# KAIST-AILab/SyncVSR

Measured on AMD Instinct MI355X. Metric: lip-clips/sec training (29x88x88), higher is better.
Workload: dtype bf16; 1 GPU; LRW training step (fwd+bwd+allreduce+clip+AdamW), ResNet18 + 6-layer 512-d encoder + vq audio-token CE head, random-init weights, N(0,1) clips 29x88x88, uniform tokens/labels; per_gpu_batch=32, global_batch=32, parallelism=dp1, hip_graph=False, enqueue=native step list

## Files before the change

include/syncvsr_hip.h:

```cpp
#ifndef SYNCVSR_HIP_H
#define SYNCVSR_HIP_H

#include <stdint.h>

#ifndef __HIP_PLATFORM_AMD__
typedef void* hipStream_t;
#else
#include <hip/hip_runtime_api.h>
#endif

#define SVSR_OK 0
#define SVSR_ERR_ARG 1001
#define SVSR_GRAD_ADD_DW 1
#define SVSR_GRAD_ADD_DB 2
#define SVSR_ERR_GROUP_OPEN 1003
#define SVSR_ERR_NO_GROUP 1004
#define SVSR_ERR_MASK_SIZE 1005

typedef struct svsr_wgrad_problem {
    const void* x; const void* dy; float* dw; float* dbias; const int* plan_dev; const int* meta;
    int Nimg; int in_pix; int Ci; int in_pitch; int Co; int out_pix; int out_pitch; int wt_taps;
} svsr_wgrad_problem;

typedef struct svsr_enc_layer {
// ... 23 lines not shown
int svsr_colsum_rows(const float* ws, int nrows, int64_t ld, float* out0, int64_t n0, float* out1, int64_t n1, int accumulate, float scale, hipStream_t stream);
int svsr_colsum_rows_multi(const void* entries, int n, hipStream_t stream);

int svsr_conv_plan(int mode, int Nimg, int H, int W, int Co_out, int k, int stride, int pad, int* words, int cap_words, int* meta);
int svsr_rows_plan(int Nimg, int P, int src0, int dst0, int Co_out, int* words, int cap_words, int* meta);
int svsr_igemm_fwd_kgroups(const int* meta, int Ci, int Co, int bn_epilogue);
int svsr_igemm_fwd(const void* in, const void* wt, void* out, void* out_pre, const float* bias, const void* addend, float* stats, const int* plan_dev, const int* meta, int Nimg, int in_pix, int Ci, int in_pitch, int Co, int out_pix, int out_pitch, int wt_taps, int act, int out_f32, float alpha, const unsigned* drop_seed, unsigned drop_site, float drop_p, hipStream_t stream);

int svsr_wgrad_plan(int Nimg, int H, int W, int Ci, int Co, int k, int stride, int pad, int* words, int cap_words, int* meta, int64_t* part_floats);
int svsr_wgrad_rows_plan(int Nimg, int P, int src0, int dst0, int Ci, int Co, int has_bias, int* words, int cap_words, int* meta, int64_t* part_floats);
int svsr_igemm_wgrad(const void* x, const void* dyp, float* dw, float* dbias, const int* plan_dev, const int* meta, int Nimg, int in_pix, int Ci, int in_pitch, int Co, int out_pix, int out_pitch, int wt_taps, float* part, int64_t part_floats, hipStream_t stream);
int svsr_wgrad_rows_plan_tile(int Nimg, int P, int src0, int dst0, int Ci, int Co, int has_bias, int bc, int* words, int cap_words, int* meta, int64_t* part_floats);
int64_t svsr_igemm_wgrad_group_bytes(int n);
int svsr_igemm_wgrad_group(const svsr_wgrad_problem* problems, int n, void* table_dev, int64_t table_bytes, hipStream_t stream);
int svsr_igemm_wgrad_v2(const void* x, const void* dyp, float* dw, float* dbias, const int* plan_dev, const int* meta, int Nimg, int in_pix, int Ci, int in_pitch, int Co, int out_pix, int out_pitch, int wt_taps, float* part, int64_t part_floats, int mode, hipStream_t stream);
int svsr_igemm_wgrad_group_v2(const svsr_wgrad_problem* problems, const int* modes, int n, void* table_dev, int64_t table_bytes, hipStream_t stream);

int svsr_conv3x3_c64_stat_rows(int Nimg, int H, int W);
int64_t svsr_conv3x3_c64_pixtab(int Nimg, int H, int W, int* out, int64_t cap);
int svsr_conv3x3_c64(const void* in, const void* wt, void* out, const void* addend, float* stats, int Nimg, int H, int W, const int* dy, const int* dx, const int* tw, const int* pixtab, hipStream_t stream);

int svsr_igemm_dgrad_bn(const void* in, const void* wt, void* out, const void* addend, float* stats, const int* plan_dev, const int* meta, int Nimg, int in_pix, int Ci, int in_pitch, int Co, int out_pix, int out_pitch, int wt_taps, const void* y, const void* x, const float* mean, const float* rstd, const float* gamma, const float* beta, int act, hipStream_t stream);
int svsr_igemm_dgrad_relu(const void* in, const void* wt, void* out, float* stats, const int* plan_dev, const int* meta, int Nimg, int in_pix, int Ci, int in_pitch, int Co, int out_pix, int out_pitch, int wt_taps, const void* y, const float* zeros, const float* ones, float gscale, hipStream_t stream);
int svsr_conv3x3_c64_dgrad_bn(const void* in, const void* wt, void* out, const void* addend, float* stats, int Nimg, int H, int W, const int* dy, const int* dx, const int* tw, const void* y, const void* x, const float* mean, const float* rstd, const float* gamma, const float* beta, int act, const int* pixtab, hipStream_t stream);
int svsr_bn_bwd_from_stats(const void* g, const void* x, const float* mean, const float* rstd, const float* gamma, const float* stats, int nrows, float* coef, float* dgamma, float* dbeta, void* dx, int64_t npix, int C, hipStream_t stream);


int svsr_conv3x3_wgrad_plan(int Nimg, int H, int W, int Ci, int Co, int* splits, int64_t* part_floats);
int svsr_conv3x3_wgrad(const void* x, const void* dy, float* dw, int Nimg, int H, int W, int Ci, int Co, float* part, int64_t part_floats, hipStream_t stream);
int svsr_conv3x3_wgrad_v2(const void* x, const void* dy, float* dw, int Nimg, int H, int W, int Ci, int Co, float* part, int64_t part_floats, int mode, hipStream_t stream);
int svsr_conv3x3_wgrad_chain(const void* x, const void* dy, float* dw, int Nimg, int H, int W, int Ci, int Co, float* part, int64_t part_floats, int mode, int defer, const float* pend_part, float* pend_dw, int pend_splits, int pend_Ci, int pend_Co, int pend_mode, hipStream_t stream);
int svsr_conv3x3_wgrad_reduce(const float* part, float* dw, int splits, int Ci, int Co, int mode, hipStream_t stream);

int svsr_stem_conv_fwd_stat_rows(int B, int T, int H, int W);
int64_t svsr_stem_conv_fwd_ws_bytes(int B, int T, int H, int W);
int svsr_stem_conv_fwd(const float* vid, const float* w, void* out, float* stats, int B, int T, int H, int W, void* ws, int64_t ws_bytes, hipStream_t stream);

int svsr_stem_conv_wgrad_plan(int B, int T, int H, int W, int* splits, int64_t* part_floats);
int svsr_stem_conv_wgrad(const float* vid, const void* dy, float* dw, int B, int T, int H, int W, int use_tr, float* part, int64_t part_floats, hipStream_t stream);

int svsr_stem_bwd_wgrad_ok(int B, int T, int H, int W);
int svsr_stem_bwd_wgrad(const float* vid, const void* gpool, const void* amax, const void* x, const float* mean, const float* rstd, const float* coef, float* dw, int B, int T, int H, int W, float* part, int64_t part_floats, hipStream_t stream);

int svsr_bn_finalize(const float* part, int nrows, int C, float count, float eps, float momentum, float* mean, float* rstd, float* running_mean, float* running_var, int64_t* num_batches_tracked, hipStream_t stream);

int svsr_bn_eval_prepare(const float* running_mean, const float* running_var, int C, float eps, float* mean, float* rstd, hipStream_t stream);
// ... 197 lines not shown
```

syncvsr_amd/csrc/igemm_fwd.h:

```cpp
#pragma once
#include "common.h"

struct IgemmFwdArgs {
    const bf16_t* in;
    const bf16_t* wt;
    void* out;
    bf16_t* out_pre;
    const float* bias;
    const bf16_t* addend;
    float* stats;
    const int* plan;
    int Nimg, in_pix, Ci, in_pitch;
    int Co, out_pix, out_pitch, wt_taps;
    int act, out_f32;
    float alpha;
    DropArgs drop;
    const bf16_t* bnb_y;
    const bf16_t* bnb_x;
    const float* bnb_mean;
    const float* bnb_rstd;
    const float* bnb_gamma;
    const float* bnb_beta;
    int bnb_act;
};


#define LDS_SWZ(row, chunk) ((row) * 64 + ((((chunk) ^ (((row) >> 1) & 7))) << 3))

#define P8_MAGIC 0x50380001
#define P8_HDR_WORDS 8
#define P8_DESC_WORDS 64
#define P8_BM 256
#define P8_BN 128
int igemm_p8_launch(const IgemmFwdArgs& a, const int* meta, hipStream_t stream);
```

syncvsr_amd/csrc/igemm_fwd.hip:

```cpp

#include <algorithm>
#include <map>
#include <vector>

#include "common.h"
#include "igemm_fwd.h"

#define PLAN_CLS_WORDS 24
#define PLAN_HDR_WORDS 2

__device__ unsigned g_zero_page[64];


template <int BM, int BN, int TM, int TN>
__device__ __forceinline__ void igemm_epilogue(const IgemmFwdArgs& p, f32x16 (&acc)[TM][TN], unsigned char* smem_raw, const long* sRow,
                                               int wm0, int wn0, int n0, int tid, bool active, int m_tile) {
    constexpr int WN = BN / 2;
    const int lane = tid & 63, wave = tid >> 6;
    float st_s[TN], st_q[TN];
    const bool bnb = p.bnb_x != nullptr;
    if (p.stats != nullptr && !bnb) {
#pragma unroll
        for (int j = 0; j < TN; ++j) {
            float s = 0.f, q = 0.f;
// ... 268 lines not shown
        for (int i = 0; i < TM; ++i)
#pragma unroll
            for (int j = 0; j < TN; ++j)
                acc[i][j] = __builtin_amdgcn_mfma_f32_32x32x16_bf16(fa[i], fb[j], acc[i][j], 0, 0, 0);
    }
}

template <int LPT, int MAXL>
__device__ __forceinline__ void wait_tiles_barrier(int later) {
    if constexpr (MAXL > 0) {
        if (later == MAXL) { SVSR_WAIT_VM_BARRIER(LPT * MAXL); return; }
        wait_tiles_barrier<LPT, MAXL - 1>(later);
    } else {
        asm volatile("s_waitcnt vmcnt(0)\n\ts_barrier" ::: "memory");
    }
}

__device__ __forceinline__ void split_row(int m, int P, float inv_p, int& n, int& j) {
    n = (int)((float)m * inv_p);
    j = m - n * P;
    if (j < 0) { n--; j += P; } else if (j >= P) { n++; j -= P; }
}

template <int BM, int BN, int NS, int KG = 1>
__global__ __launch_bounds__(256 * KG) void k_igemm_fwd_glds(const IgemmFwdArgs p) {
    constexpr int BK = 64;
    static_assert(NS >= 2 && (BM / 32 + BN / 32) * (NS - 2) <= 63, "vmcnt immediate is 6 bits");
    constexpr int WM = BM / 2, WN = BN / 2, TM = WM / 32, TN = WN / 32;
    constexpr int A_ELEMS = BM * BK, B_ELEMS = BN * BK, S_ELEMS = A_ELEMS + B_ELEMS;
    constexpr int AR = BM / 32, BR = BN / 32, LPT = AR + BR;
    extern __shared__ __attribute__((aligned(16))) unsigned char smem_raw[];
    const int grp = KG == 1 ? 0 : __builtin_amdgcn_readfirstlane((int)threadIdx.x >> 8);
    bf16_t* sStage = reinterpret_cast<bf16_t*>(smem_raw) + grp * NS * S_ELEMS;
    long* sRow = reinterpret_cast<long*>(reinterpret_cast<bf16_t*>(smem_raw) + KG * NS * S_ELEMS);
    int* sTap = reinterpret_cast<int*>(sRow + BM);

    const int tid = threadIdx.x & 255, lane = tid & 63, wave = tid >> 6;
    const int wm0 = (wave >> 1) * WM, wn0 = (wave & 1) * WN;
    const int bx = blockIdx.x, by = blockIdx.y;
    const int n0 = by * BN;
    const int slot = tid & 7, r0 = tid >> 3;
    const int csw = slot ^ ((r0 >> 1) & 7);
    const int wrow = __builtin_amdgcn_readfirstlane(wave) * 8;

    const int hdr0 = p.plan[0];
    const int ncls = hdr0 & 0xffff;
    const bool identity = (hdr0 >> 16) != 0;
// ... 32 lines not shown
    }
    for (int r = tid; r < BM; r += 256) {
        const int m = m0 + r;
        long off = -1;
        if (m < Mc) {
            if (identity) {
                off = (long)m * p.out_pix * p.out_pitch;
            } else {
                int n, j;
                split_row(m, P, inv_p, n, j);
                off = ((long)n * p.out_pix + pos[2 * j + 1]) * p.out_pitch;
            }
        }
        sRow[r] = off;
    }
    __syncthreads();

    const int KT_all = ntaps * (p.Ci / BK);
    const int KT_loop = (KT_all + KG - 1) / KG;
    const int k_begin = grp * KT_loop;
    const int KT = KT_all - k_begin < KT_loop ? (KT_all - k_begin > 0 ? KT_all - k_begin : 0) : KT_loop;
    const int spt = p.Ci / BK;
    int t_next = k_begin / spt, c_next = (k_begin - (k_begin / spt) * spt) * BK;
    auto stage = [&](int buf) {
        const int tw = sTap[9 + t_next];
        const int c0 = c_next;
        const long a_off = (long)sTap[t_next] * p.in_pitch + c0;
        bf16_t* dstA = sStage + buf * S_ELEMS + wrow * 64;
#pragma unroll
        for (int i = 0; i < AR; ++i) {
            const bf16_t* src = ((a_ok >> i) & 1u) ? a_ptr[i] + a_off : zero_src;
            __builtin_amdgcn_global_load_lds((const __attribute__((address_space(1))) void*)src,
                                             (__attribute__((address_space(3))) void*)(dstA + i * 32 * 64), 16, 0, 0);
        }
        bf16_t* dstB = sStage + buf * S_ELEMS + A_ELEMS + wrow * 64;
#pragma unroll
        for (int i = 0; i < BR; ++i) {
            const bf16_t* src = b_ptr[i] != nullptr ? b_ptr[i] + (long)tw * p.Ci + c0 : zero_src;
            __builtin_amdgcn_global_load_lds((const __attribute__((address_space(1))) void*)src,
                                             (__attribute__((address_space(3))) void*)(dstB + i * 32 * 64), 16, 0, 0);
        }
        c_next += BK;
        if (c_next >= p.Ci) { c_next = 0; ++t_next; }
    };

    f32x16 acc[TM][TN];
#pragma unroll
    for (int i = 0; i < TM; ++i)
#pragma unroll
        for (int j = 0; j < TN; ++j)
#pragma unroll
            for (int r = 0; r < 16; ++r) acc[i][j][r] = 0.f;

#pragma unroll
    for (int s = 0; s < NS - 1; ++s)
        if (s < KT) stage(s);
    int buf = 0;
    for (int it = 0; it < KT_loop; ++it) {
        int later = KT - 1 - it < NS - 2 ? KT - 1 - it : NS - 2;
        if (later < 0) later = 0;
        wait_tiles_barrier<LPT, NS - 2>(later);
        if (it + NS - 1 < KT) stage(buf >= 1 ? buf - 1 : NS - 1);
        if (KG == 1 || it < KT) {
            const bf16_t* cA = sStage + buf * S_ELEMS;
            igemm_mma_tile<BM, BN, TM, TN>(cA, cA + A_ELEMS, acc, wm0, wn0, lane);
        }
// ... 5 lines not shown
        static_assert((size_t)TM * TN * 16 * 256 * sizeof(float) <= (size_t)NS * S_ELEMS * sizeof(bf16_t), "exchange buffer fits the ring");
        if (grp == 1) {
#pragma unroll
            for (int i = 0; i < TM; ++i)
#pragma unroll
                for (int j = 0; j < TN; ++j)
#pragma unroll
                    for (int r = 0; r < 16; ++r) sX[((i * TN + j) * 16 + r) * 256 + tid] = acc[i][j][r];
        }
        __syncthreads();
        if (grp == 0) {
#pragma unroll
            for (int i = 0; i < TM; ++i)
#pragma unroll
                for (int j = 0; j < TN; ++j)
#pragma unroll
                    for (int r = 0; r < 16; ++r) acc[i][j][r] += sX[((i * TN + j) * 16 + r) * 256 + tid];
        }
        __syncthreads();
    }
    igemm_epilogue<BM, BN, TM, TN>(p, acc, smem_raw, sRow, wm0, wn0, n0, tid, grp == 0, bx);
}

template <int BM, int BN, int NS, int KG = 1>
static int launch_glds(const IgemmFwdArgs& a, int gx, int gy, hipStream_t stream) {
    const size_t lds = (size_t)KG * NS * (BM + BN) * 64 * sizeof(bf16_t) + (size_t)BM * sizeof(long) + 128;
    static size_t attr_set = 0;
    if (attr_set < lds) {
        (void)hipFuncSetAttribute(reinterpret_cast<const void*>(k_igemm_fwd_glds<BM, BN, NS, KG>), hipFuncAttributeMaxDynamicSharedMemorySize, (int)lds);
        attr_set = lds;
    }
    IgemmFwdArgs b = a;
    hipLaunchKernelGGL((k_igemm_fwd_glds<BM, BN, NS, KG>), dim3(gx, gy), dim3(256 * KG), lds, stream, b);
    return svsr_check_launch();
}

struct IgemmFwdPlan { int bm, bn, ns, gy; };

static IgemmFwdPlan igemm_fwd_plan(long M, int Co, int max_taps) {
    const int cus = svsr_stream_cus(nullptr);
    IgemmFwdPlan pl;
    const int forced = svsr_tune_get(SVSR_TUNE_IGEMM_TILE);
    const int thr = svsr_tune_get(SVSR_TUNE_IGEMM_M128);
    int bm;
    if (forced == 64 || forced == 128) bm = forced;
    else if (Co <= 64) bm = M >= 16384 ? 128 : 64;
    else {
        const long blocks128 = ((M + 127) / 128) * ((Co + 127) / 128);
        bm = (M >= thr || blocks128 >= 224) ? 128 : 64;
    }
    const int lin_rows = svsr_tune_get(SVSR_TUNE_IGEMM_LIN_BN64);
    if (bm == 64 && forced == 0 && Co > 64 && max_taps == 1 && lin_rows > 0 && M >= lin_rows) { pl.bm = 128; pl.bn = 64; pl.ns = 3; }
    else if (bm == 128 && Co > 64 && max_taps > 1 && ((M + 127) / 128) * ((Co + 127) / 128) < svsr_tune_get(SVSR_TUNE_IGEMM_BN64_BELOW)) { pl.bm = 128; pl.bn = 64; pl.ns = 2; }
    else if (bm == 128 && Co <= 64) { pl.bm = 128; pl.bn = 64; pl.ns = max_taps <= 4 ? 2 : 3; }
    else if (bm == 128) { pl.bm = 128; pl.bn = 128; pl.ns = 2; }
    else { pl.bm = 64; pl.bn = 64; pl.ns = 0; }
// ... 72 lines not shown
            const PlanClass& c = cls[i];
            int* w = words + PLAN_HDR_WORDS + i * PLAN_CLS_WORDS;
            const int P = (int)(c.pos.size() / 2);
            if ((long)Nimg * P >= (1L << 24)) return -SVSR_ERR_ARG;
            w[0] = c.ntaps; w[1] = P; w[2] = pos_off; w[3] = (int)tiles;
            for (int t = 0; t < 9; ++t) { w[4 + t] = t < c.ntaps ? c.delta[t] : 0; w[13 + t] = t < c.ntaps ? c.tw[t] : 0; }
            w[22] = 0; w[23] = 0;
            std::copy(c.pos.begin(), c.pos.end(), words + pos_word0 + 2 * pos_off);
            pos_off += P;
            tiles += ((long)Nimg * P + pl.bm - 1) / pl.bm;
        }
    } else {
        for (const PlanClass& c : cls) tiles += ((long)Nimg * (long)(c.pos.size() / 2) + pl.bm - 1) / pl.bm;
    }
    if (tiles > 0x7fffffffL) return -SVSR_ERR_ARG;
    if (meta != nullptr) {
        meta[0] = pl.bm; meta[1] = pl.bn; meta[2] = pl.ns; meta[3] = (int)tiles; meta[4] = pl.gy; meta[5] = ncls; meta[6] = max_taps;
        meta[7] = (int)(M & 0x7fffffff);
    }
    return nwords;
}

extern "C" int svsr_conv_plan(int mode, int Nimg, int H, int W, int Co_out, int k, int stride, int pad, int* words, int cap_words, int* meta) {
    if (Nimg < 1 || H < 1 || W < 1 || k < 1 || k > 3 || stride < 1 || pad < 0 || Co_out < 1 || mode < 0 || mode > 2) return -SVSR_ERR_ARG;
    const int Ho = (H + 2 * pad - k) / stride + 1, Wo = (W + 2 * pad - k) / stride + 1;
    if (Ho < 1 || Wo < 1) return -SVSR_ERR_ARG;
    std::vector<PlanClass> cls;
    std::map<std::vector<int>, int> index;
    auto add = [&](const std::vector<int>& key, int src, int dst) {
        auto it = index.find(key);
        if (it == index.end()) {
            PlanClass c;
            c.ntaps = (int)(key.size() / 2);
            for (int t = 0; t < c.ntaps; ++t) { c.delta[t] = key[2 * t]; c.tw[t] = key[2 * t + 1]; }
            cls.push_back(c);
            it = index.emplace(key, (int)cls.size() - 1).first;
        }
        cls[it->second].pos.push_back(src);
        cls[it->second].pos.push_back(dst);
    };
    std::vector<int> key;
    if (mode == 0) {
        for (int a = 0; a < Ho; ++a)
            for (int b = 0; b < Wo; ++b) {
                key.clear();
                for (int kh = 0; kh < k; ++kh)
                    for (int kw = 0; kw < k; ++kw) {
                        const int iy = a * stride + kh - pad, ix = b * stride + kw - pad;
                        if (iy < 0 || iy >= H || ix < 0 || ix >= W) continue;
                        key.push_back((kh - pad) * W + (kw - pad));
                        key.push_back(kh * k + kw);
                    }
                add(key, (a * stride) * W + b * stride, a * Wo + b);
            }
    } else {
        for (int y = 0; y < H; ++y)
            for (int x = 0; x < W; ++x) {
                key.clear();
                const int a = y / stride, b = x / stride, py = y % stride, px = x % stride;
                for (int kh = 0; kh < k; ++kh) {
                    if ((py + pad - kh) % stride) continue;
                    for (int kw = 0; kw < k; ++kw) {
                        if ((px + pad - kw) % stride) continue;
                        const int dq = (py + pad - kh) / stride, dp = (px + pad - kw) / stride;
                        const int oy = a + dq, ox = b + dp;
                        if (oy < 0 || oy >= Ho || ox < 0 || ox >= Wo) continue;
                        key.push_back(dq * Wo + dp);
                        key.push_back(kh * k + kw);
                    }
                }
                int ca = a < Ho ? a : Ho - 1, cb = b < Wo ? b : Wo - 1;
                if (ca != a || cb != b) {
                    const int shift = (a - ca) * Wo + (b - cb);
                    for (size_t t = 0; t < key.size(); t += 2) key[t] += shift;
                }
                if (mode == 2 && key.empty()) continue;
                add(key, ca * Wo + cb, y * W + x);
            }
    }
    const int p8_pix[2] = {mode == 0 ? H * W : Ho * Wo, mode == 0 ? Ho * Wo : H * W};
    const bool p8_ok = k == 3 && pad == 1 && H >= 2 && W >= 2 && (stride == 1 || (stride == 2 && mode == 0 && svsr_tune_get(SVSR_TUNE_P8) >= 1 && svsr_tune_get(SVSR_TUNE_P8) != 3));
    return plan_emit(cls, Nimg, Co_out, words, cap_words, meta, p8_ok ? p8_pix : nullptr);
}

extern "C" int svsr_rows_plan(int Nimg, int P, int src0, int dst0, int Co_out, int* words, int cap_words, int* meta) {
    if (Nimg < 1 || P < 1 || Co_out < 1) return -SVSR_ERR_ARG;
    std::vector<PlanClass> cls(1);
    cls[0].ntaps = 1; cls[0].delta[0] = 0; cls[0].tw[0] = 0;
    cls[0].pos.reserve(2 * (size_t)P);
    for (int j = 0; j < P; ++j) { cls[0].pos.push_back(src0 + j); cls[0].pos.push_back(dst0 + j); }
    const int n = plan_emit(cls, Nimg, Co_out, words, cap_words, meta);
    if (n > 0 && words != nullptr && P == 1 && src0 == 0 && dst0 == 0) words[0] |= 1 << 16;
    return n;
}

extern "C" int svsr_igemm_fwd_kgroups(const int* meta, int Ci, int Co, int bn_epilogue) {
    if (meta == nullptr || Ci < 64) return 1;
    const int bm = meta[0], bn = meta[1], gx = meta[3], gy = (Co + bn - 1) / bn;
    const int ks = svsr_tune_get(SVSR_TUNE_IGEMM_KSPLIT);
    if (!bn_epilogue && bm == 64 && bn == 64 && ks && (long)gx * gy <= ks && (long)meta[6] * (Ci / 64) >= 12) return 2;
    const int ks128 = svsr_tune_get(SVSR_TUNE_IGEMM_KSPLIT128);
    if (!bn_epilogue && bm == 128 && bn == 64 && meta[2] == 3 && meta[6] == 1 && ks128 > 0 && Ci / 64 >= ks128 && (long)gx * gy <= 288) return 2;
    return 1;
}

static int igemm_fwd_run(const void* in, const void* wt, void* out, void* out_pre, const float* bias, const void* addend,
                         float* stats, const int* plan_dev, const int* meta, int Nimg, int in_pix, int Ci, int in_pitch, int Co,
                         int out_pix, int out_pitch, int wt_taps, int act, int out_f32, float alpha, const unsigned* drop_seed,
                         unsigned drop_site, float drop_p, const void* bnb_y, const void* bnb_x, const float* bnb_mean,
                         const float* bnb_rstd, const float* bnb_gamma, const float* bnb_beta, int bnb_act, hipStream_t stream) {
    if (plan_dev == nullptr || meta == nullptr || Ci % 64 != 0 || Ci <= 0 || Co <= 0 || in_pitch % 8 != 0 || Nimg <= 0 || wt_taps < 1)
        return SVSR_ERR_ARG;
    if (act != 0 && (addend != nullptr || alpha != 1.f)) return SVSR_ERR_ARG;
    IgemmFwdArgs a;
    a.in = (const bf16_t*)in; a.wt = (const bf16_t*)wt; a.out = out; a.out_pre = (bf16_t*)out_pre;
    a.bias = bias; a.addend = (const bf16_t*)addend; a.stats = stats; a.plan = plan_dev;
    a.Nimg = Nimg; a.in_pix = in_pix; a.Ci = Ci; a.in_pitch = in_pitch; a.Co = Co; a.out_pix = out_pix; a.out_pitch = out_pitch;
    a.wt_taps = wt_taps; a.act = act; a.out_f32 = out_f32; a.alpha = alpha;
    a.drop = svsr_make_drop(drop_seed, drop_site, drop_p);
    a.bnb_y = (const bf16_t*)bnb_y; a.bnb_x = (const bf16_t*)bnb_x; a.bnb_mean = bnb_mean; a.bnb_rstd = bnb_rstd;
    a.bnb_gamma = bnb_gamma; a.bnb_beta = bnb_beta; a.bnb_act = bnb_act;
    const int bm = meta[0], bn = meta[1], ns = meta[2], gx = meta[3], gy = (Co + bn - 1) / bn;
    if (gx < 1) return SVSR_ERR_ARG;
    if (bm == P8_BM) return (bnb_x != nullptr && alpha != 1.f) ? SVSR_ERR_ARG : igemm_p8_launch(a, meta, stream);
    if (svsr_igemm_fwd_kgroups(meta, Ci, Co, bnb_x != nullptr) == 2) {
        if (bm == 128) return launch_glds<128, 64, 3, 2>(a, gx, gy, stream);
        return launch_glds<64, 64, 4, 2>(a, gx, gy, stream);
    }
#define SVSR_IGEMM_CASE(BM_, BN_, NS_) if (bm == BM_ && bn == BN_ && ns == NS_) return launch_glds<BM_, BN_, NS_>(a, gx, gy, stream)
    SVSR_IGEMM_CASE(128, 128, 2);
    SVSR_IGEMM_CASE(128, 64, 2);
    SVSR_IGEMM_CASE(128, 64, 3);
    SVSR_IGEMM_CASE(64, 64, 4);
    SVSR_IGEMM_CASE(64, 64, 3);
#undef SVSR_IGEMM_CASE
    return SVSR_ERR_ARG;
}

extern "C" int svsr_igemm_fwd(const void* in, const void* wt, void* out, void* out_pre, const float* bias, const void* addend,
                              float* stats, const int* plan_dev, const int* meta, int Nimg, int in_pix, int Ci, int in_pitch, int Co,
                              int out_pix, int out_pitch, int wt_taps, int act, int out_f32, float alpha, const unsigned* drop_seed,
                              unsigned drop_site, float drop_p, hipStream_t stream) {
    return igemm_fwd_run(in, wt, out, out_pre, bias, addend, stats, plan_dev, meta, Nimg, in_pix, Ci, in_pitch, Co, out_pix, out_pitch,
                         wt_taps, act, out_f32, alpha, drop_seed, drop_site, drop_p, nullptr, nullptr, nullptr, nullptr, nullptr, nullptr, 0, stream);
}

extern "C" int svsr_igemm_dgrad_relu(const void* in, const void* wt, void* out, float* stats, const int* plan_dev, const int* meta, int Nimg,
                                     int in_pix, int Ci, int in_pitch, int Co, int out_pix, int out_pitch, int wt_taps, const void* y,
                                     const float* zeros, const float* ones, float gscale, hipStream_t stream) {
    if (y == nullptr || zeros == nullptr || ones == nullptr || stats == nullptr || Co % 8 != 0 || out_pitch % 8 != 0 || !(gscale > 0.f)) return SVSR_ERR_ARG;
    return igemm_fwd_run(in, wt, out, nullptr, nullptr, nullptr, stats, plan_dev, meta, Nimg, in_pix, Ci, in_pitch, Co, out_pix, out_pitch,
                         wt_taps, 0, 0, gscale, nullptr, 0, 0.f, nullptr, y, zeros, ones, ones, zeros, 1, stream);
}

extern "C" int svsr_igemm_dgrad_bn(const void* in, const void* wt, void* out, const void* addend, float* stats, const int* plan_dev,
                                   const int* meta, int Nimg, int in_pix, int Ci, int in_pitch, int Co, int out_pix, int out_pitch,
                                   int wt_taps, const void* y, const void* x, const float* mean, const float* rstd, const float* gamma,
                                   const float* beta, int act, hipStream_t stream) {
    if (x == nullptr || mean == nullptr || rstd == nullptr || stats == nullptr || Co % 8 != 0 || out_pitch % 8 != 0) return SVSR_ERR_ARG;
    if (act != 1 && act != 2) return SVSR_ERR_ARG;
    if ((y == nullptr || act == 2) && (gamma == nullptr || beta == nullptr)) return SVSR_ERR_ARG;
    return igemm_fwd_run(in, wt, out, nullptr, nullptr, addend, stats, plan_dev, meta, Nimg, in_pix, Ci, in_pitch, Co, out_pix, out_pitch,
                         wt_taps, 0, 0, 1.0f, nullptr, 0, 0.f, y, x, mean, rstd, gamma, beta, act, stream);
}
```

syncvsr_amd/csrc/steplist.hip:

```cpp
#include <stdlib.h>
#include <string.h>

#include <string>
#include <unordered_map>
#include <utility>
#include <vector>

#include "common.h"
#include "../../include/syncvsr_hip.h"

namespace {

typedef int64_t Slot;

template <typename T> struct FromSlot;
template <> struct FromSlot<int> { static int get(Slot s) { return (int)s; } };
template <> struct FromSlot<unsigned> { static unsigned get(Slot s) { return (unsigned)s; } };
template <> struct FromSlot<int64_t> { static int64_t get(Slot s) { return s; } };
template <> struct FromSlot<float> { static float get(Slot s) { double d; memcpy(&d, &s, sizeof d); return (float)d; } };
template <typename P> struct FromSlot<P*> { static P* get(Slot s) { return reinterpret_cast<P*>((uintptr_t)s); } };

template <typename... A, size_t... I>
int invoke(int (*fn)(A...), const Slot* s, std::index_sequence<I...>) { return fn(FromSlot<A>::get(s[I])...); }

template <typename... A>
int thunk_n(int (*)(A...)) { return (int)sizeof...(A); }

typedef int (*Thunk)(const Slot*);
struct Entry { Thunk call; int nargs; };

template <typename F, F fn> struct Bind;
template <typename... A, int (*fn)(A...)>
struct Bind<int (*)(A...), fn> {
    static int call(const Slot* s) { return invoke(fn, s, std::index_sequence_for<A...>{}); }
    static constexpr int nargs = (int)sizeof...(A);
};

#define SVSR_REG(f) {#f, Entry{&Bind<decltype(&f), &f>::call, Bind<decltype(&f), &f>::nargs}}

const std::unordered_map<std::string, Entry>& registry() {
    static const std::unordered_map<std::string, Entry> r = {
        SVSR_REG(svsr_colsum_rows), SVSR_REG(svsr_colsum_rows_multi), SVSR_REG(svsr_igemm_fwd), SVSR_REG(svsr_igemm_wgrad), SVSR_REG(svsr_conv3x3_c64),
        SVSR_REG(svsr_igemm_dgrad_bn), SVSR_REG(svsr_igemm_dgrad_relu), SVSR_REG(svsr_conv3x3_c64_dgrad_bn), SVSR_REG(svsr_bn_bwd_from_stats),
        SVSR_REG(svsr_conv3x3_wgrad), SVSR_REG(svsr_stem_conv_fwd), SVSR_REG(svsr_stem_conv_wgrad), SVSR_REG(svsr_stem_bwd_wgrad), SVSR_REG(svsr_bn_finalize),
        SVSR_REG(svsr_bn_eval_prepare), SVSR_REG(svsr_bn_act_fwd), SVSR_REG(svsr_bn_act_bwd), SVSR_REG(svsr_stem_bn_act_pool_fwd),
        SVSR_REG(svsr_stem_bn_act_pool_bwd), SVSR_REG(svsr_avgpool_fwd), SVSR_REG(svsr_avgpool_bwd), SVSR_REG(svsr_add_ln_fwd),
        SVSR_REG(svsr_add_ln_bwd), SVSR_REG(svsr_embed_ln_fwd), SVSR_REG(svsr_embed_bwd_scatter), SVSR_REG(svsr_rmsnorm_fwd),
        SVSR_REG(svsr_rmsnorm_bwd), SVSR_REG(svsr_rotary), SVSR_REG(svsr_geglu_fwd), SVSR_REG(svsr_geglu_bwd), SVSR_REG(svsr_xt_embed_fwd),
        SVSR_REG(svsr_xt_embed_bwd), SVSR_REG(svsr_bias_act_bwd), SVSR_REG(svsr_ce_fwd), SVSR_REG(svsr_ce_bwd), SVSR_REG(svsr_linear_ce_fwd), SVSR_REG(svsr_linear_ce_bwd), SVSR_REG(svsr_topk_acc),
        SVSR_REG(svsr_grad_sumsq), SVSR_REG(svsr_grad_sumsq_parts), SVSR_REG(svsr_adamw_step), SVSR_REG(svsr_adamw_range), SVSR_REG(svsr_cast_bf16), SVSR_REG(svsr_transpose_cast_multi),
        SVSR_REG(svsr_transpose_bf16_multi), SVSR_REG(svsr_fill_f32), SVSR_REG(svsr_clip_prep), SVSR_REG(svsr_mha_fwd), SVSR_REG(svsr_mha_bwd), SVSR_REG(svsr_mha_flash_fwd), SVSR_REG(svsr_mha_flash_bwd), SVSR_REG(svsr_mha_flash_bwd_parts), SVSR_REG(svsr_mha_pe_transpose),
        SVSR_REG(svsr_glu_dwconv_fwd), SVSR_REG(svsr_glu_dwconv_bwd), SVSR_REG(svsr_glu_dwconv_bwd_parts), SVSR_REG(svsr_ctc_fwd), SVSR_REG(svsr_ctc_grad),
        SVSR_REG(svsr_ctc_prefix_score), SVSR_REG(svsr_lrs_targets), SVSR_REG(svsr_embed_pos_fwd), SVSR_REG(svsr_embed_pos_bwd), SVSR_REG(svsr_ls_loss_fwd),
        SVSR_REG(svsr_ls_loss_bwd), SVSR_REG(svsr_scale_bf16), SVSR_REG(svsr_word_add), SVSR_REG(svsr_lincomb2), SVSR_REG(svsr_igemm_wgrad_group), SVSR_REG(svsr_enc_fwd), SVSR_REG(svsr_enc_bwd), SVSR_REG(svsr_lincomb3_ratio), SVSR_REG(svsr_add_ln_bwd_partials), SVSR_REG(svsr_add_ln_bwd_branch), SVSR_REG(svsr_bias_act_bwd_partials),
        SVSR_REG(svsr_memcpy_async), SVSR_REG(svsr_w2v_conv0), SVSR_REG(svsr_w2v_norm_gelu), SVSR_REG(svsr_w2v_quantize),
        SVSR_REG(svsr_igemm_wgrad_v2), SVSR_REG(svsr_igemm_wgrad_group_v2), SVSR_REG(svsr_conv3x3_wgrad_v2), SVSR_REG(svsr_fill_ranges),
        SVSR_REG(svsr_conv3x3_wgrad_chain), SVSR_REG(svsr_conv3x3_wgrad_reduce),
        SVSR_REG(svsr_mha_table_fwd), SVSR_REG(svsr_lm_embed_fwd),
        SVSR_REG(svsr_beam_select), SVSR_REG(svsr_ctc_prefix_score_clips), SVSR_REG(svsr_mha_src_step_fwd), SVSR_REG(svsr_ctc_align),
        SVSR_REG(svsr_ctc_frame_best), SVSR_REG(svsr_ctc_collapse), SVSR_REG(svsr_edit_distance),
        SVSR_REG(svsr_tconv_fwd), SVSR_REG(svsr_tcn_se_fwd), SVSR_REG(svsr_tcn_norm_pool_fwd),
        SVSR_REG(svsr_tconv_fwd_save), SVSR_REG(svsr_tconv_epi_bwd), SVSR_REG(svsr_tconv_dgrad), SVSR_REG(svsr_tconv_wgrad), SVSR_REG(svsr_tcn_se_bwd),
        SVSR_REG(svsr_tcn_norm_pool_bwd), SVSR_REG(svsr_tcn_fold),
        SVSR_REG(svsr_tconv_fwd_ext), SVSR_REG(svsr_tcn_colstats), SVSR_REG(svsr_tconv_apply), SVSR_REG(svsr_tconv_epi_bwd_bs), SVSR_REG(svsr_tconv_bn_bwd),
        SVSR_REG(svsr_tconv_dgrad_ext), SVSR_REG(svsr_tconv_wgrad_ext), SVSR_REG(svsr_tcn_norm_pool_bwd_bs),
        SVSR_REG(svsr_lrs_clip_prep), SVSR_REG(svsr_wave_prep),
// ... 261 lines not shown
```

syncvsr_amd/model.py:

```python
from __future__ import annotations

import math
from typing import Any, Optional

import torch
import torch.nn as nn

from . import ops
from .config import Config, audio_codec_dims
from .init import buffer_specs, hidden_dim, init_state_dict, pad64, param_specs, phys_shape, resnet_block_specs, xt_dims

BF16 = torch.bfloat16


class _SideStream:

    def __init__(self) -> None:
        self.stream: Optional[torch.cuda.Stream] = None
        self.keep: list = []
        self._issuing = False
        self.enabled = False
        self.enabled_small = False

    def run(self, fn, *keep, small: bool = False, behind_main: bool = True) -> None:
# ... 691 lines not shown
        if fused:
            g1, st1 = ops.conv2d_dgrad_bn(dc2, w2t, 3, 1, 1, t2["x"].shape[1:3], None, None, t1["c"], t1["mean"], t1["rstd"],
                                          st.p32(f"{t1['bn']}.weight"), st.p32(f"{t1['bn']}.bias"), act)
            dc1 = ops.bn_bwd_from_stats(g1, t1["c"], t1["mean"], t1["rstd"], st.p32(f"{t1['bn']}.weight"), st1, ws1["coef"],
                                        st.g32(f"{t1['bn']}.weight"), st.g32(f"{t1['bn']}.bias"))
        else:
            do1 = ops.conv2d_dgrad(dc2, w2t, 3, 1, 1, t2["x"].shape[1:3])
            dc1, _ = ops.bn_act_bwd(do1, t1["y"], t1["c"], t1["mean"], t1["rstd"], st.p32(f"{t1['bn']}.weight"), ws1["coef"],
                                    st.g32(f"{t1['bn']}.weight"), st.g32(f"{t1['bn']}.bias"), act, False, beta=st.p32(f"{t1['bn']}.bias"))
        _conv_wgrad(model, st, f"{prefix}.conv1", t1, dc1)
        in_hw = t1["x"].shape[1:3]
        w1t = st.t16(f"{prefix}.conv1.weight").view(inp, 3, 3, planes)
        tp = tape[f"{blocks[bi - 1][0]}.conv2"] if fused and bi > 0 else None
        if tp is not None:
            tp_aux = tp["y"] if act == 1 else tp["res"]
            tp_gb = (st.p32(f"{tp['bn']}.weight"), st.p32(f"{tp['bn']}.bias"), act)
        if down:
            td = tape[f"{prefix}.downsample.0"]
            wsd = st.bn[td["bn"]]
            dcd, _ = ops.bn_act_bwd(dres, None, td["c"], td["mean"], td["rstd"], st.p32(f"{td['bn']}.weight"), wsd["coef"],
                                    st.g32(f"{td['bn']}.weight"), st.g32(f"{td['bn']}.bias"), 0, False)
            _conv_wgrad(model, st, f"{prefix}.downsample.0", td, dcd)
            wdt = st.t16(f"{prefix}.downsample.0.weight").view(inp, 1, 1, planes)
            dxd = ops.conv2d_dgrad(dcd, wdt, 1, stride, 0, in_hw)
            if tp is not None:
                dx, dx_stats = ops.conv2d_dgrad_bn(dc1, w1t, 3, stride, 1, in_hw, dxd, tp_aux, tp["c"], tp["mean"], tp["rstd"], *tp_gb)
            else:
                dx, dx_stats = ops.conv2d_dgrad(dc1, w1t, 3, stride, 1, in_hw, addend=dxd), None
        elif tp is not None:
            dx, dx_stats = ops.conv2d_dgrad_bn(dc1, w1t, 3, stride, 1, in_hw, dres, tp_aux, tp["c"], tp["mean"], tp["rstd"], *tp_gb)
        else:
            dx, dx_stats = ops.conv2d_dgrad(dc1, w1t, 3, stride, 1, in_hw, addend=dres), None
        _ready(model, st, f"{prefix}.conv1.weight")
    _flush_w3_chain(model)
    ts = tape["stem"]
    if rec is not None:
        rec["stem"] = (dx.clone(), False)
    sc, sb = model.stem_name + ".0", model.stem_name + ".1"
    ws = st.bn[sb]
    fused = ts.get("xwin") is not None and ops.stem_bwd_wgrad_ok(ts["videos"])
    dconv = ops.stem_bn_gelu_pool_bwd(dx, ts["amax"], ts["c"], ts["mean"], ts["rstd"], st.p32(f"{sb}.weight"), st.p32(f"{sb}.bias"),
                                      ws["coef"], st.g32(f"{sb}.weight"), st.g32(f"{sb}.bias"), model.stem_act, xwin=ts.get("xwin"),
                                      want_dx=not fused)
    if fused:
        _flush_deferred(model)
        model._side.join()
        early = model._early_sumsq
        if early is not None and st.sumsq_head:
            with ops.window_group("tail"):
                model._side.run(lambda: ops.grad_sumsq_parts(st.grad, st.sumsq_head, st.numel - st.sumsq_head, early, 0, ops.SUMSQ_PARTS - 1))
            st.sumsq_tail_done = True
# ... 500 lines not shown
```

syncvsr_amd/ops.py:

```python
from __future__ import annotations

import bisect
import ctypes
import os
import struct
from contextlib import contextmanager, nullcontext
from typing import Callable, Optional, Sequence

import torch

from . import _lib

BF16 = torch.bfloat16
BN_EPS = 1e-5
BN_MOMENTUM = 0.1
HALO_WGRAD = True


_DEV_INDEX: Optional[int] = None
STREAM_OVERRIDE: Optional[int] = None


def _stream() -> int:
    global _DEV_INDEX
# ... 748 lines not shown
                    addend: Optional[torch.Tensor], y: Optional[torch.Tensor], x: torch.Tensor, mean: torch.Tensor, rstd: torch.Tensor,
                    gamma: Optional[torch.Tensor] = None, beta: Optional[torch.Tensor] = None, act: int = 1):
    N, Ho, Wo, Co = dy.shape
    Ci = w16t.shape[0]
    H, W = in_hw
    if x.shape != (N, H, W, Ci) or not x.is_contiguous() or (y is not None and (y.shape != x.shape or not y.is_contiguous())):
        raise ValueError("conv2d_dgrad_bn: y / x must be contiguous tensors with the geometry of the result")
    if (y is None or act == 2) and (gamma is None or beta is None):
        raise ValueError("conv2d_dgrad_bn: y=None / act=2 need gamma and beta")
    g = torch.empty((N, H, W, Ci), dtype=BF16, device=dy.device) if addend is None else addend
    if stride == 1 and _c64_ok(Ci, Co, k, stride, pad, W):
        taps = tuple((pad - kh, pad - kw, kh * k + kw) for kh in range(k) for kw in range(k))
        tdy, tdx, tw = zip(*taps)
        rows = _query("svsr_conv3x3_c64_stat_rows", N, H, W)[0]
        stats = scratch(rows * 2 * 64)
        _call("svsr_conv3x3_c64_dgrad_bn", _p(dy), _p(w16t), _p(g), _p(addend), _p(stats), N, H, W, _ints(tdy), _ints(tdx), _ints(tw),
              _p(y), _p(x), _p(mean), _p(rstd), _p(gamma), _p(beta), act, _p(c64_pixtab(N, H, W, dy.device)), _stream(), label="k_conv3x3_c64+bn", flops=2.0 * N * H * W * 64 * 64 * 9)
        return g, (stats, rows)
    plan = conv_plan(1, N, H, W, Ci, k, stride, pad)
    stats = scratch(plan.tiles * 2 * Ci)
    _call("svsr_igemm_dgrad_bn", _p(dy), _p(w16t), _p(g), _p(addend), _p(stats), plan.words.data_ptr(), plan.meta, N, Ho * Wo, Co, Co, Ci,
          H * W, Ci, k * k, _p(y), _p(x), _p(mean), _p(rstd), _p(gamma), _p(beta), act, _stream(), label=plan.label + "+bn", flops=2.0 * N * Ho * Wo * Co * Ci * k * k)
    return g, (stats, plan.tiles)


def bn_bwd_from_stats(g, x, mean, rstd, gamma, stats, coef, dgamma, dbeta) -> torch.Tensor:
    part, rows = stats
    C = x.shape[-1]
    dx = torch.empty_like(x)
    _call("svsr_bn_bwd_from_stats", _p(g), _p(x), _p(mean), _p(rstd), _p(gamma), _p(part), rows, _p(coef), _p(dgamma), _p(dbeta), _p(dx),
          x.numel() // C, C, _stream())
    return dx


def conv2d_wgrad(x: torch.Tensor, dy: torch.Tensor, dw: torch.Tensor, k: int, stride: int, pad: int, use_tr: bool = True, mode: Optional[int] = None) -> None:
    N, H, W, Ci = x.shape
    _, Ho, Wo, Co = dy.shape
    if HALO_WGRAD and use_tr and k == 3 and stride == 1 and pad == 1 and W <= 29 and H * W >= 100 and Ci % 64 == 0 and Co % 64 == 0:
        _, nfl = _query("svsr_conv3x3_wgrad_plan", N, H, W, Ci, Co)
        part = scratch(nfl) if nfl else None
        _call("svsr_conv3x3_wgrad_v2", _p(x), _p(dy), _p(dw), N, H, W, Ci, Co, _p(part), nfl, _grad_add(dw, Co * 9 * Ci) if mode is None else mode & 1, _stream(),
              label="k_wgrad3x3_halo", flops=2.0 * N * H * W * Co * Ci * 9)
        return
    igemm_wgrad(wgrad_conv_plan(N, H, W, Ci, Co, k, stride, pad), x, dy, dw, Nimg=N, in_pix=H * W, Ci=Ci, in_pitch=Ci, Co=Co,
                out_pix=Ho * Wo, out_pitch=Co, wt_taps=k * k, flops=2.0 * N * Ho * Wo * Co * Ci * k * k, mode=mode)

# ... 1518 lines not shown
```

Baseline: 7120 clips/s.

## Fuse downsample 1x1 dgrad into strided 3x3 dgrad as a tenth tap

For stride-2 residual blocks, the 1x1 downsample conv's data-gradient is folded into the 3x3 conv's dgrad implicit GEMM. A new plan mode adds an extra tap that reads the downsample gradient and weight, so both contributions accumulate in one kernel. This removes a separate dgrad launch, the intermediate dxd tensor and its re-read as an addend. In exchange it adds templated kernel variants with pointer-offset arithmetic for the second operand, plus extra per-tap branching in the staging loop.

```diff
diff --git a/include/syncvsr_hip.h b/include/syncvsr_hip.h
--- a/include/syncvsr_hip.h
+++ b/include/syncvsr_hip.h
@@ -69,6 +69,8 @@
 
 int svsr_igemm_dgrad_bn(const void* in, const void* wt, void* out, const void* addend, float* stats, const int* plan_dev, const int* meta, int Nimg, int in_pix, int Ci, int in_pitch, int Co, int out_pix, int out_pitch, int wt_taps, const void* y, const void* x, const float* mean, const float* rstd, const float* gamma, const float* beta, int act, hipStream_t stream);
 int svsr_igemm_dgrad_relu(const void* in, const void* wt, void* out, float* stats, const int* plan_dev, const int* meta, int Nimg, int in_pix, int Ci, int in_pitch, int Co, int out_pix, int out_pitch, int wt_taps, const void* y, const float* zeros, const float* ones, float gscale, hipStream_t stream);
+int svsr_igemm_dgrad2(const void* in, const void* wt, const void* in2, const void* wt2, void* out, void* out_pre, const float* bias, float* stats, const int* plan_dev, const int* meta, int Nimg, int in_pix, int Ci, int in_pitch, int Co, int out_pix, int out_pitch, int wt_taps, int act, int out_f32, float alpha, const unsigned* drop_seed, unsigned drop_site, float drop_p, hipStream_t stream);
+int svsr_igemm_dgrad2_bn(const void* in, const void* wt, const void* in2, const void* wt2, void* out, float* stats, const int* plan_dev, const int* meta, int Nimg, int in_pix, int Ci, int in_pitch, int Co, int out_pix, int out_pitch, int wt_taps, const void* y, const void* x, const float* mean, const float* rstd, const float* gamma, const float* beta, int act, hipStream_t stream);
 int svsr_conv3x3_c64_dgrad_bn(const void* in, const void* wt, void* out, const void* addend, float* stats, int Nimg, int H, int W, const int* dy, const int* dx, const int* tw, const void* y, const void* x, const float* mean, const float* rstd, const float* gamma, const float* beta, int act, const int* pixtab, hipStream_t stream);
 int svsr_bn_bwd_from_stats(const void* g, const void* x, const float* mean, const float* rstd, const float* gamma, const float* stats, int nrows, float* coef, float* dgamma, float* dbeta, void* dx, int64_t npix, int C, hipStream_t stream);
 
diff --git a/syncvsr_amd/csrc/igemm_fwd.h b/syncvsr_amd/csrc/igemm_fwd.h
--- a/syncvsr_amd/csrc/igemm_fwd.h
+++ b/syncvsr_amd/csrc/igemm_fwd.h
@@ -22,7 +22,11 @@
     const float* bnb_gamma;
     const float* bnb_beta;
     int bnb_act;
+    const bf16_t* in2;
+    const bf16_t* wt2;
 };
+
+#define IGEMM_TAP2 9
 
 
 #define LDS_SWZ(row, chunk) ((row) * 64 + ((((chunk) ^ (((row) >> 1) & 7))) << 3))
diff --git a/syncvsr_amd/csrc/igemm_fwd.hip b/syncvsr_amd/csrc/igemm_fwd.hip
--- a/syncvsr_amd/csrc/igemm_fwd.hip
+++ b/syncvsr_amd/csrc/igemm_fwd.hip
@@ -314,7 +314,7 @@
     if (j < 0) { n--; j += P; } else if (j >= P) { n++; j -= P; }
 }
 
-template <int BM, int BN, int NS, int KG = 1>
+template <int BM, int BN, int NS, int KG = 1, bool TWO = false>
 __global__ __launch_bounds__(256 * KG) void k_igemm_fwd_glds(const IgemmFwdArgs p) {
     constexpr int BK = 64;
     static_assert(NS >= 2 && (BM / 32 + BN / 32) * (NS - 2) <= 63, "vmcnt immediate is 6 bits");
@@ -393,10 +393,29 @@
     const int KT = KT_all - k_begin < KT_loop ? (KT_all - k_begin > 0 ? KT_all - k_begin : 0) : KT_loop;
     const int spt = p.Ci / BK;
     int t_next = k_begin / spt, c_next = (k_begin - (k_begin / spt) * spt) * BK;
+    long a_tap = 0, b_tap = 0, b_rows = 0;
+    const long in2_off = TWO ? (reinterpret_cast<intptr_t>(p.in2) - reinterpret_cast<intptr_t>(p.in)) / (long)sizeof(bf16_t) : 0;
+    const long b2_rows = TWO ? -32L * (p.wt_taps - 1) * p.Ci : 0;
+    const long b2_lane = TWO ? (reinterpret_cast<intptr_t>(p.wt2) - reinterpret_cast<intptr_t>(p.wt)) / (long)sizeof(bf16_t) - (long)(n0 + r0) * (p.wt_taps - 1) * p.Ci : 0;
+    auto enter_tap = [&]() {
+        if (t_next >= 9) return;
+        const int tw = __builtin_amdgcn_readfirstlane(sTap[9 + t_next]);
+        const bool second = tw == IGEMM_TAP2;
+        a_tap = (long)sTap[t_next] * p.in_pitch + (second ? in2_off : 0);
+        b_tap = second ? b2_lane : (long)tw * p.Ci;
+        b_rows = second ? b2_rows : 0;
+    };
+    if constexpr (TWO) enter_tap();
     auto stage = [&](int buf) {
-        const int tw = sTap[9 + t_next];
         const int c0 = c_next;
-        const long a_off = (long)sTap[t_next] * p.in_pitch + c0;
+        long a_off, b_off;
+        if constexpr (TWO) {
+            a_off = a_tap + c0;
+            b_off = b_tap + c0;
+        } else {
+            a_off = (long)sTap[t_next] * p.in_pitch + c0;
+            b_off = (long)sTap[9 + t_next] * p.Ci + c0;
+        }
         bf16_t* dstA = sStage + buf * S_ELEMS + wrow * 64;
 #pragma unroll
         for (int i = 0; i < AR; ++i) {
@@ -407,12 +426,15 @@
         bf16_t* dstB = sStage + buf * S_ELEMS + A_ELEMS + wrow * 64;
 #pragma unroll
         for (int i = 0; i < BR; ++i) {
-            const bf16_t* src = b_ptr[i] != nullptr ? b_ptr[i] + (long)tw * p.Ci + c0 : zero_src;
+            const bf16_t* src = b_ptr[i] != nullptr ? b_ptr[i] + b_off + (TWO ? i * b_rows : 0) : zero_src;
             __builtin_amdgcn_global_load_lds((const __attribute__((address_space(1))) void*)src,
                                              (__attribute__((address_space(3))) void*)(dstB + i * 32 * 64), 16, 0, 0);
         }
         c_next += BK;
-        if (c_next >= p.Ci) { c_next = 0; ++t_next; }
+        if (c_next >= p.Ci) {
+            c_next = 0; ++t_next;
+            if constexpr (TWO) enter_tap();
+        }
     };
 
     f32x16 acc[TM][TN];
@@ -464,16 +486,16 @@
     igemm_epilogue<BM, BN, TM, TN>(p, acc, smem_raw, sRow, wm0, wn0, n0, tid, grp == 0, bx);
 }
 
-template <int BM, int BN, int NS, int KG = 1>
+template <int BM, int BN, int NS, int KG = 1, bool TWO = false>
 static int launch_glds(const IgemmFwdArgs& a, int gx, int gy, hipStream_t stream) {
     const size_t lds = (size_t)KG * NS * (BM + BN) * 64 * sizeof(bf16_t) + (size_t)BM * sizeof(long) + 128;
     static size_t attr_set = 0;
     if (attr_set < lds) {
-        (void)hipFuncSetAttribute(reinterpret_cast<const void*>(k_igemm_fwd_glds<BM, BN, NS, KG>), hipFuncAttributeMaxDynamicSharedMemorySize, (int)lds);
+        (void)hipFuncSetAttribute(reinterpret_cast<const void*>(k_igemm_fwd_glds<BM, BN, NS, KG, TWO>), hipFuncAttributeMaxDynamicSharedMemorySize, (int)lds);
         attr_set = lds;
     }
     IgemmFwdArgs b = a;
-    hipLaunchKernelGGL((k_igemm_fwd_glds<BM, BN, NS, KG>), dim3(gx, gy), dim3(256 * KG), lds, stream, b);
+    hipLaunchKernelGGL((k_igemm_fwd_glds<BM, BN, NS, KG, TWO>), dim3(gx, gy), dim3(256 * KG), lds, stream, b);
     return svsr_check_launch();
 }
 
@@ -592,7 +614,8 @@
 }
 
 extern "C" int svsr_conv_plan(int mode, int Nimg, int H, int W, int Co_out, int k, int stride, int pad, int* words, int cap_words, int* meta) {
-    if (Nimg < 1 || H < 1 || W < 1 || k < 1 || k > 3 || stride < 1 || pad < 0 || Co_out < 1 || mode < 0 || mode > 2) return -SVSR_ERR_ARG;
+    if (Nimg < 1 || H < 1 || W < 1 || k < 1 || k > 3 || stride < 1 || pad < 0 || Co_out < 1 || mode < 0 || mode > 3) return -SVSR_ERR_ARG;
+    if (mode == 3 && (k != 3 || stride != 2 || pad != 1)) return -SVSR_ERR_ARG;
     const int Ho = (H + 2 * pad - k) / stride + 1, Wo = (W + 2 * pad - k) / stride + 1;
     if (Ho < 1 || Wo < 1) return -SVSR_ERR_ARG;
     std::vector<PlanClass> cls;
@@ -637,6 +660,10 @@
                         if (oy < 0 || oy >= Ho || ox < 0 || ox >= Wo) continue;
                         key.push_back(dq * Wo + dp);
                         key.push_back(kh * k + kw);
+                        if (mode == 3 && kh == 1 && kw == 1) {
+                            key.push_back(dq * Wo + dp);
+                            key.push_back(IGEMM_TAP2);
+                        }
                     }
                 }
                 int ca = a < Ho ? a : Ho - 1, cb = b < Wo ? b : Wo - 1;
@@ -678,9 +705,11 @@
                          float* stats, const int* plan_dev, const int* meta, int Nimg, int in_pix, int Ci, int in_pitch, int Co,
                          int out_pix, int out_pitch, int wt_taps, int act, int out_f32, float alpha, const unsigned* drop_seed,
                          unsigned drop_site, float drop_p, const void* bnb_y, const void* bnb_x, const float* bnb_mean,
-                         const float* bnb_rstd, const float* bnb_gamma, const float* bnb_beta, int bnb_act, hipStream_t stream) {
+                         const float* bnb_rstd, const float* bnb_gamma, const float* bnb_beta, int bnb_act, hipStream_t stream,
+                         const void* in2 = nullptr, const void* wt2 = nullptr) {
     if (plan_dev == nullptr || meta == nullptr || Ci % 64 != 0 || Ci <= 0 || Co <= 0 || in_pitch % 8 != 0 || Nimg <= 0 || wt_taps < 1)
         return SVSR_ERR_ARG;
+    if ((in2 == nullptr) != (wt2 == nullptr)) return SVSR_ERR_ARG;
     if (act != 0 && (addend != nullptr || alpha != 1.f)) return SVSR_ERR_ARG;
     IgemmFwdArgs a;
     a.in = (const bf16_t*)in; a.wt = (const bf16_t*)wt; a.out = out; a.out_pre = (bf16_t*)out_pre;
@@ -690,8 +719,19 @@
     a.drop = svsr_make_drop(drop_seed, drop_site, drop_p);
     a.bnb_y = (const bf16_t*)bnb_y; a.bnb_x = (const bf16_t*)bnb_x; a.bnb_mean = bnb_mean; a.bnb_rstd = bnb_rstd;
     a.bnb_gamma = bnb_gamma; a.bnb_beta = bnb_beta; a.bnb_act = bnb_act;
+    a.in2 = (const bf16_t*)in2; a.wt2 = (const bf16_t*)wt2;
     const int bm = meta[0], bn = meta[1], ns = meta[2], gx = meta[3], gy = (Co + bn - 1) / bn;
     if (gx < 1) return SVSR_ERR_ARG;
+    if (in2 != nullptr) {
+        if (bm == 64 && bn == 64 && svsr_igemm_fwd_kgroups(meta, Ci, Co, bnb_x != nullptr) == 2) return launch_glds<64, 64, 4, 2, true>(a, gx, gy, stream);
+#define SVSR_IGEMM_CASE2(BM_, BN_, NS_) if (bm == BM_ && bn == BN_ && ns == NS_) return launch_glds<BM_, BN_, NS_, 1, true>(a, gx, gy, stream)
+        SVSR_IGEMM_CASE2(128, 128, 2);
+        SVSR_IGEMM_CASE2(128, 64, 2);
+        SVSR_IGEMM_CASE2(64, 64, 4);
+        SVSR_IGEMM_CASE2(64, 64, 3);
+#undef SVSR_IGEMM_CASE2
+        return SVSR_ERR_ARG;
+    }
     if (bm == P8_BM) return (bnb_x != nullptr && alpha != 1.f) ? SVSR_ERR_ARG : igemm_p8_launch(a, meta, stream);
     if (svsr_igemm_fwd_kgroups(meta, Ci, Co, bnb_x != nullptr) == 2) {
         if (bm == 128) return launch_glds<128, 64, 3, 2>(a, gx, gy, stream);
@@ -733,3 +773,25 @@
     return igemm_fwd_run(in, wt, out, nullptr, nullptr, addend, stats, plan_dev, meta, Nimg, in_pix, Ci, in_pitch, Co, out_pix, out_pitch,
                          wt_taps, 0, 0, 1.0f, nullptr, 0, 0.f, y, x, mean, rstd, gamma, beta, act, stream);
 }
+
+extern "C" int svsr_igemm_dgrad2(const void* in, const void* wt, const void* in2, const void* wt2, void* out, void* out_pre, const float* bias,
+                                 float* stats, const int* plan_dev, const int* meta, int Nimg, int in_pix, int Ci, int in_pitch, int Co,
+                                 int out_pix, int out_pitch, int wt_taps, int act, int out_f32, float alpha, const unsigned* drop_seed,
+                                 unsigned drop_site, float drop_p, hipStream_t stream) {
+    if (in2 == nullptr || wt2 == nullptr) return SVSR_ERR_ARG;
+    return igemm_fwd_run(in, wt, out, out_pre, bias, nullptr, stats, plan_dev, meta, Nimg, in_pix, Ci, in_pitch, Co, out_pix, out_pitch,
+                         wt_taps, act, out_f32, alpha, drop_seed, drop_site, drop_p, nullptr, nullptr, nullptr, nullptr, nullptr, nullptr, 0, stream,
+                         in2, wt2);
+}
+
+extern "C" int svsr_igemm_dgrad2_bn(const void* in, const void* wt, const void* in2, const void* wt2, void* out, float* stats, const int* plan_dev,
+                                    const int* meta, int Nimg, int in_pix, int Ci, int in_pitch, int Co, int out_pix, int out_pitch,
+                                    int wt_taps, const void* y, const void* x, const float* mean, const float* rstd, const float* gamma,
+                                    const float* beta, int act, hipStream_t stream) {
+    if (in2 == nullptr || wt2 == nullptr) return SVSR_ERR_ARG;
+    if (x == nullptr || mean == nullptr || rstd == nullptr || stats == nullptr || Co % 8 != 0 || out_pitch % 8 != 0) return SVSR_ERR_ARG;
+    if (act != 1 && act != 2) return SVSR_ERR_ARG;
+    if ((y == nullptr || act == 2) && (gamma == nullptr || beta == nullptr)) return SVSR_ERR_ARG;
+    return igemm_fwd_run(in, wt, out, nullptr, nullptr, nullptr, stats, plan_dev, meta, Nimg, in_pix, Ci, in_pitch, Co, out_pix, out_pitch,
+                         wt_taps, 0, 0, 1.0f, nullptr, 0, 0.f, y, x, mean, rstd, gamma, beta, act, stream, in2, wt2);
+}
diff --git a/syncvsr_amd/csrc/steplist.hip b/syncvsr_amd/csrc/steplist.hip
--- a/syncvsr_amd/csrc/steplist.hip
+++ b/syncvsr_amd/csrc/steplist.hip
@@ -41,7 +41,7 @@
 const std::unordered_map<std::string, Entry>& registry() {
     static const std::unordered_map<std::string, Entry> r = {
         SVSR_REG(svsr_colsum_rows), SVSR_REG(svsr_colsum_rows_multi), SVSR_REG(svsr_igemm_fwd), SVSR_REG(svsr_igemm_wgrad), SVSR_REG(svsr_conv3x3_c64),
-        SVSR_REG(svsr_igemm_dgrad_bn), SVSR_REG(svsr_igemm_dgrad_relu), SVSR_REG(svsr_conv3x3_c64_dgrad_bn), SVSR_REG(svsr_bn_bwd_from_stats),
+        SVSR_REG(svsr_igemm_dgrad_bn), SVSR_REG(svsr_igemm_dgrad_relu), SVSR_REG(svsr_igemm_dgrad2), SVSR_REG(svsr_igemm_dgrad2_bn), SVSR_REG(svsr_conv3x3_c64_dgrad_bn), SVSR_REG(svsr_bn_bwd_from_stats),
         SVSR_REG(svsr_conv3x3_wgrad), SVSR_REG(svsr_stem_conv_fwd), SVSR_REG(svsr_stem_conv_wgrad), SVSR_REG(svsr_stem_bwd_wgrad), SVSR_REG(svsr_bn_finalize),
         SVSR_REG(svsr_bn_eval_prepare), SVSR_REG(svsr_bn_act_fwd), SVSR_REG(svsr_bn_act_bwd), SVSR_REG(svsr_stem_bn_act_pool_fwd),
         SVSR_REG(svsr_stem_bn_act_pool_bwd), SVSR_REG(svsr_avgpool_fwd), SVSR_REG(svsr_avgpool_bwd), SVSR_REG(svsr_add_ln_fwd),
diff --git a/syncvsr_amd/model.py b/syncvsr_amd/model.py
--- a/syncvsr_amd/model.py
+++ b/syncvsr_amd/model.py
@@ -737,11 +737,17 @@
                                     st.g32(f"{td['bn']}.weight"), st.g32(f"{td['bn']}.bias"), 0, False)
             _conv_wgrad(model, st, f"{prefix}.downsample.0", td, dcd)
             wdt = st.t16(f"{prefix}.downsample.0.weight").view(inp, 1, 1, planes)
-            dxd = ops.conv2d_dgrad(dcd, wdt, 1, stride, 0, in_hw)
-            if tp is not None:
-                dx, dx_stats = ops.conv2d_dgrad_bn(dc1, w1t, 3, stride, 1, in_hw, dxd, tp_aux, tp["c"], tp["mean"], tp["rstd"], *tp_gb)
+            if ops.DGRAD2 and stride == 2:
+                if tp is not None:
+                    dx, dx_stats = ops.conv2d_dgrad2(dc1, w1t, dcd, wdt, in_hw, bn=(tp_aux, tp["c"], tp["mean"], tp["rstd"], *tp_gb))
+                else:
+                    dx, dx_stats = ops.conv2d_dgrad2(dc1, w1t, dcd, wdt, in_hw), None
             else:
-                dx, dx_stats = ops.conv2d_dgrad(dc1, w1t, 3, stride, 1, in_hw, addend=dxd), None
+                dxd = ops.conv2d_dgrad(dcd, wdt, 1, stride, 0, in_hw)
+                if tp is not None:
+                    dx, dx_stats = ops.conv2d_dgrad_bn(dc1, w1t, 3, stride, 1, in_hw, dxd, tp_aux, tp["c"], tp["mean"], tp["rstd"], *tp_gb)
+                else:
+                    dx, dx_stats = ops.conv2d_dgrad(dc1, w1t, 3, stride, 1, in_hw, addend=dxd), None
         elif tp is not None:
             dx, dx_stats = ops.conv2d_dgrad_bn(dc1, w1t, 3, stride, 1, in_hw, dres, tp_aux, tp["c"], tp["mean"], tp["rstd"], *tp_gb)
         else:
diff --git a/syncvsr_amd/ops.py b/syncvsr_amd/ops.py
--- a/syncvsr_amd/ops.py
+++ b/syncvsr_amd/ops.py
@@ -794,6 +794,35 @@
     _call("svsr_igemm_dgrad_bn", _p(dy), _p(w16t), _p(g), _p(addend), _p(stats), plan.words.data_ptr(), plan.meta, N, Ho * Wo, Co, Co, Ci,
           H * W, Ci, k * k, _p(y), _p(x), _p(mean), _p(rstd), _p(gamma), _p(beta), act, _stream(), label=plan.label + "+bn", flops=2.0 * N * Ho * Wo * Co * Ci * k * k)
     return g, (stats, plan.tiles)
+
+
+DGRAD2 = True
+
+
+def conv2d_dgrad2(dy: torch.Tensor, w16t: torch.Tensor, dy2: torch.Tensor, w16t2: torch.Tensor, in_hw: tuple[int, int], bn: Optional[tuple] = None):
+    N, Ho, Wo, Co = dy.shape
+    Ci = w16t.shape[0]
+    H, W = in_hw
+    if dy2.shape != dy.shape or not (dy.is_contiguous() and dy2.is_contiguous()) or w16t2.numel() != Ci * Co or w16t.numel() != Ci * 9 * Co:
+        raise ValueError("conv2d_dgrad2: dy2 must have dy's shape, the weights must be [Ci][3][3][Co] and [Ci][Co]")
+    plan = conv_plan(3, N, H, W, Ci, 3, 2, 1)
+    dx = torch.empty((N, H, W, Ci), dtype=BF16, device=dy.device)
+    flops = 2.0 * N * Ho * Wo * Co * Ci * 10
+    head = (_p(dy), _p(w16t), _p(dy2), _p(w16t2), _p(dx))
+    label = plan.label[:-1] + ",1,true>"
+    if bn is None:
+        _call("svsr_igemm_dgrad2", *head, None, None, None, plan.words.data_ptr(), plan.meta, N, Ho * Wo, Co, Co, Ci, H * W, Ci, 9, 0, 0, 1.0,
+              *_drop(None), _stream(), label=label, flops=flops)
+        return dx
+    y, x, mean, rstd, gamma, beta, act = bn
+    if x.shape != dx.shape or not x.is_contiguous() or (y is not None and (y.shape != x.shape or not y.is_contiguous())):
+        raise ValueError("conv2d_dgrad2: y / x must be contiguous tensors with the geometry of the result")
+    if (y is None or act == 2) and (gamma is None or beta is None):
+        raise ValueError("conv2d_dgrad2: y=None / act=2 need gamma and beta")
+    stats = scratch(plan.tiles * 2 * Ci)
+    _call("svsr_igemm_dgrad2_bn", *head, _p(stats), plan.words.data_ptr(), plan.meta, N, Ho * Wo, Co, Co, Ci, H * W, Ci, 9, _p(y), _p(x),
+          _p(mean), _p(rstd), _p(gamma), _p(beta), act, _stream(), label=label + "+bn", flops=flops)
+    return dx, (stats, plan.tiles)
 
 
 def bn_bwd_from_stats(g, x, mean, rstd, gamma, stats, coef, dgamma, dbeta) -> torch.Tensor:
```

Measured after the change: 7223 clips/s (median of 6 runs). 1.4% higher.
